# casper-hansen/AutoAWQ

Measured on NVIDIA H100. Metric: decode tok/s Llama-3-8B W4A16 (quantised linears, bs=1, seq=1), higher is better.
Workload: dtype f16

## Files before the change

### autoawq_b200/csrc/common.cuh

```cuda
#pragma once
#include <cuda_fp16.h>
#include <cuda_runtime.h>
#include <stdint.h>

namespace b200awq {

#ifndef B200AWQ_SM_COUNT_FALLBACK
#define B200AWQ_SM_COUNT_FALLBACK 132
#endif

__device__ __forceinline__ uint32_t smem_u32(const void* p) {
  return static_cast<uint32_t>(__cvta_generic_to_shared(p));
}
__device__ __forceinline__ uint32_t lane_id() { return threadIdx.x & 31; }

__device__ __forceinline__ bool elect_one() {
  uint32_t pred;
  asm volatile(
      "{\n\t.reg .pred p;\n\telect.sync _|p, 0xffffffff;\n\tselp.u32 %0, 1, 0, p;\n\t}\n"
      : "=r"(pred));
  return pred != 0;
}

__device__ __forceinline__ uint4 ldg_stream_u4(const void* p) {
// ... 154 lines not shown
  asm volatile("prefetch.tensormap [%0];" ::"l"(tmap) : "memory");
}
__device__ __forceinline__ void tma_load_2d(void* smem_dst, const void* tmap, uint64_t* bar, int c0, int c1) {
  asm volatile(
      "cp.async.bulk.tensor.2d.shared::cluster.global.mbarrier::complete_tx::bytes [%0], [%1, {%3, %4}], [%2];"
      ::"r"(smem_u32(smem_dst)), "l"(tmap), "r"(smem_u32(bar)), "r"(c0), "r"(c1)
      : "memory");
}
__device__ __forceinline__ void tma_prefetch_l2_2d(const void* tmap, int c0, int c1) {
  asm volatile("cp.async.bulk.prefetch.tensor.2d.L2.global [%0, {%1, %2}];" ::"l"(tmap), "r"(c0), "r"(c1) : "memory");
}
__device__ __forceinline__ void prefetch_l2_line(const void* gsrc) {
  asm volatile("prefetch.global.L2 [%0];" ::"l"(gsrc) : "memory");
}
__device__ __forceinline__ void bulk_prefetch_l2(const void* gsrc, uint32_t bytes) {
  asm volatile("cp.async.bulk.prefetch.L2.global [%0], %1;" ::"l"(gsrc), "r"(bytes) : "memory");
}
__device__ __forceinline__ void bulk_load_1d(void* smem_dst, const void* gsrc, uint32_t bytes, uint64_t* bar) {
  asm volatile(
      "cp.async.bulk.shared::cluster.global.mbarrier::complete_tx::bytes [%0], [%1], %2, [%3];"
      ::"r"(smem_u32(smem_dst)), "l"(gsrc), "r"(bytes), "r"(smem_u32(bar))
      : "memory");
}

__device__ __forceinline__ void wgmma_fence() { asm volatile("wgmma.fence.sync.aligned;" ::: "memory"); }
__device__ __forceinline__ void wgmma_commit() { asm volatile("wgmma.commit_group.sync.aligned;" ::: "memory"); }
template <int N>
__device__ __forceinline__ void wgmma_wait() { asm volatile("wgmma.wait_group.sync.aligned %0;" ::"n"(N) : "memory"); }

__device__ __forceinline__ uint64_t gmma_desc(uint32_t smem_addr, uint32_t lbo_bytes, uint32_t sbo_bytes) {
  uint64_t d = 0;
  d |= static_cast<uint64_t>((smem_addr & 0x3FFFFu) >> 4);
  d |= static_cast<uint64_t>((lbo_bytes >> 4) & 0x3FFFu) << 16;
  d |= static_cast<uint64_t>((sbo_bytes >> 4) & 0x3FFFu) << 32;
  d |= static_cast<uint64_t>(1) << 62;
  return d;
}

template <int TA>
__device__ __forceinline__ void wgmma_m64n16k16(float (&d)[8], uint64_t da, uint64_t db) {
  asm volatile(
      "wgmma.mma_async.sync.aligned.m64n16k16.f32.f16.f16 "
      "{%0, %1, %2, %3, %4, %5, %6, %7}, "
      "%8, %9, 1, 1, 1, %10, 0;"
      : "+f"(d[0]), "+f"(d[1]), "+f"(d[2]), "+f"(d[3]), "+f"(d[4]), "+f"(d[5]), "+f"(d[6]), "+f"(d[7])
      : "l"(da), "l"(db), "n"(TA)
// ... 44 lines not shown
```

### autoawq_b200/csrc/program.cu

```cuda
#include <algorithm>
#include <cstring>
#include <vector>

#include "../../include/b200awq.h"
#include "common.cuh"
#include "gemv_tile.cuh"
#include "kernels.h"
#include "rope.cuh"

namespace b200awq {

enum { kProCopy = 0, kProRmsnorm = 1, kProSilu = 2 };

struct ProgOp {
  const __half* scales;
  const int32_t* qzeros;
  const __half* bias;
  __half* y;
  const __half* src;
  const __half* norm_w;
  __half* xout;
  int src_off;
  int src_prev;
  int K, N, G;
// ... 68 lines not shown
  while (!mbar_try_wait(bar, parity))
    if (wd.tick(code, op)) return false;
  return true;
}

}
#include "program_stream.cuh"
#include "program_batch.cuh"
namespace b200awq {

struct Program {
  int n_ops = 0;
  int M = 0;
  size_t xs_bytes = 0;
  int device = 0;
  SpOp* d_sp_ops = nullptr;
  uint8_t* d_stream = nullptr;
  uint32_t* d_cta = nullptr;
  uint32_t* d_rows = nullptr;
  int* d_state = nullptr;
  int row_stride = 0;
  size_t stream_bytes = 0;
  int sb_spw = 0, sb_lmax = 0, sb_nu_max = 0;
  SpMoe* d_moe = nullptr;
  int n_moe = 0;
  SpRes* d_res = nullptr;
  SpRope* d_rope = nullptr;
};

struct ResFold {
  const void* raw_y = nullptr;
  const void* ext = nullptr;
  int op = -1;
};

struct MoeFold {
  int kind = 0;
  int mi = -1;
};

int moe_plan(int E, int topk, int H, int I, int G, int grid, int* out8) {
  if (E <= 0 || topk <= 0 || topk > E || H <= 0 || I <= 0 || G <= 0 || grid <= 0 || out8 == nullptr)
    return B200AWQ_EINVAL;
  if (E > kSpMoeEMax || topk > kSpMoeKMax) return B200AWQ_EUNSUPPORTED;
  if (!stream_format_supported(H, 2 * I, G, 1) || !stream_format_supported(I, H, G, 0)) return B200AWQ_EUNSUPPORTED;
  const int UK = G < 128 ? G : 128;
// ... 10 lines not shown
  out8[1] = sets_a;
  out8[2] = (2 * I / 16) * nu_a;
  out8[3] = lmax_a;
  out8[4] = topk * nu_b1;
  out8[5] = nu_b1;
  out8[6] = lmax_b;
  out8[7] = (int)smem;
  return B200AWQ_OK;
}

size_t stream_format_bytes(int K, int N, int G) {
  if (K <= 0 || N <= 0 || G <= 0) return 0;
  const int UK = G < 128 ? G : 128;
  return (size_t)(N / 16) * (K / UK) * ((size_t)(UK / 16) * 128 + kSpAux);
}
bool stream_format_supported(int K, int N, int G, int mode) {
  if (K <= 0 || N <= 0 || G <= 0 || (K % G) != 0 || (N % 16) != 0 || (K % 128) != 0) return false;
  if (!(G == 32 || G == 64 || (G % 128) == 0)) return false;
  if (mode == 1 && ((N / 2) % 8) != 0) return false;
  return mode == 0 || mode == 1;
}
static int prog_sm_count();

cudaError_t stream_pack_rotary(const int32_t* qweight, const void* scales, const int32_t* qzeros, void* out, int K, int N,
                               int G, int head_dim, cudaStream_t st) {
  if (!stream_format_supported(K, N, G, 0) || head_dim <= 0 || (head_dim % 16) != 0 || (N % head_dim) != 0)
    return cudaErrorNotSupported;
  const int UK = G < 128 ? G : 128;
  const int64_t total = (int64_t)(N / 16) * (K / UK) * ((UK / 16) * 32 + 12);
  const int cap = prog_sm_count() * 16;
  const int blocks = (int)((total + 255) / 256 < cap ? (total + 255) / 256 : cap);
  stream_pack_rotary_kernel<<<blocks, 256, 0, st>>>(qweight, static_cast<const __half*>(scales), qzeros,
                                                    static_cast<uint8_t*>(out), K, N, G, head_dim);
  return cudaGetLastError();
}

cudaError_t stream_pack(const int32_t* qweight, const void* scales, const int32_t* qzeros, void* out, int K, int N, int G,
                        int mode, cudaStream_t st) {
  if (!stream_format_supported(K, N, G, mode)) return cudaErrorNotSupported;
  const int UK = G < 128 ? G : 128;
  const int64_t total = (int64_t)(N / 16) * (K / UK) * ((UK / 16) * 32 + 12);
  const int cap = prog_sm_count() * 16;
  const int blocks = (int)((total + 255) / 256 < cap ? (total + 255) / 256 : cap);
  stream_pack_kernel<<<blocks, 256, 0, st>>>(qweight, static_cast<const __half*>(scales), qzeros,
                                             static_cast<uint8_t*>(out), K, N, G, mode);
  return cudaGetLastError();
// ... 47 lines not shown
      has_res = true;
    }
  size_t wbytes = 0, max_cols = 0;
  int max_K = 0, lmax = 0, nu_max = 0;
  std::vector<size_t> woff(n);
  for (int i = 0; i < n; ++i) {
    const ProgOp& p = table[i];
    if (moe_kind(i) != 0) {
      woff[i] = wbytes;
      wbytes += (size_t)moes[fold[i].mi].E * expert_bytes(i);
    } else {
      if (!stream_format_supported(p.K, p.N, p.G, mode[i] == 2 ? 0 : mode[i])) return false;
      const int UK = p.G < 128 ? p.G : 128;
      if (p.K / UK > kSpXsumMax) return false;
      if (M == 1 && (p.N / 16 + grid - 1) / grid > kSpLMax) return false;
      lmax = std::max(lmax, (p.N / 16 + grid - 1) / grid);
      nu_max = std::max(nu_max, p.K / UK);
      woff[i] = wbytes;
      wbytes += (stream_format_bytes(p.K, p.N, p.G) + 255) & ~(size_t)255;
    }
    max_cols = std::max(max_cols, (size_t)(mode[i] == 1 ? p.N / 2 : p.N));
    max_K = std::max(max_K, p.K);
  }
  if (M == 1 && (has_moe || has_res || has_rope)) {
    if (sp_fixed_smem(8, 4, true) + (size_t)max_K * 2 > (size_t)227 * 1024) return false;
  } else if (M == 1) {
    if (sp_fixed_smem(12, 3) + (size_t)max_K * 2 > (size_t)227 * 1024) return false;
  } else {
    int spw = kSbMaxStages;
    while (spw > 0 && sb_fixed_smem(spw, lmax, sb_mt(M), nu_max) + (size_t)max_K * sb_mt(M) * 2 > (size_t)227 * 1024) --spw;
    if (spw == 0) return false;
    pr->sb_spw = spw;
    pr->sb_lmax = lmax;
    pr->sb_nu_max = nu_max;
  }
  for (int i = 0; i < n; ++i) {
    const ProgOp& p = table[i];
    SpOp& o = ops[i];
    std::memset(&o, 0, sizeof(o));
    o.bias = p.bias;
    o.y = (!res.empty() && res[i].raw_y != nullptr) ? static_cast<__half*>(const_cast<void*>(res[i].raw_y)) : p.y;
    o.K = p.K;
    o.N = p.N;
    const int UK = p.G < 128 ? p.G : 128;
    o.uk_shift = UK == 32 ? 5 : (UK == 64 ? 6 : 7);
    o.F = UK / 16;
    o.NU = p.K / UK;
    o.unit_bytes = o.F * 128 + kSpAux;
    o.ups = kSpStageBytes / o.unit_bytes;
    o.mode = mode[i];
// ... 126 lines not shown
      e = cudaFuncSetAttribute(stream_batch_residual_kernel<2>, cudaFuncAttributeMaxDynamicSharedMemorySize, (int)(227 * 1024));
    if (e == cudaSuccess)
      e = cudaFuncSetAttribute(stream_batch_residual_kernel<4>, cudaFuncAttributeMaxDynamicSharedMemorySize, (int)(227 * 1024));
    if (e == cudaSuccess)
      e = cudaFuncSetAttribute(stream_batch_residual_kernel<8>, cudaFuncAttributeMaxDynamicSharedMemorySize, (int)(227 * 1024));
  }
  if (e == cudaSuccess && has_rope) {
    std::vector<SpRope> rp(n);
    for (int i = 0; i < n; ++i) rp[i].r = ropes[i];
    e = cudaMalloc(&pr->d_rope, (size_t)n * sizeof(SpRope));
    if (e == cudaSuccess) e = cudaMemcpy(pr->d_rope, rp.data(), (size_t)n * sizeof(SpRope), cudaMemcpyHostToDevice);
    if (e == cudaSuccess)
      e = cudaFuncSetAttribute(stream_rope_kernel, cudaFuncAttributeMaxDynamicSharedMemorySize, (int)(227 * 1024));
    if (e == cudaSuccess)
      e = cudaFuncSetAttribute(stream_batch_rope_kernel<2>, cudaFuncAttributeMaxDynamicSharedMemorySize, (int)(227 * 1024));
    if (e == cudaSuccess)
      e = cudaFuncSetAttribute(stream_batch_rope_kernel<4>, cudaFuncAttributeMaxDynamicSharedMemorySize, (int)(227 * 1024));
    if (e == cudaSuccess)
      e = cudaFuncSetAttribute(stream_batch_rope_kernel<8>, cudaFuncAttributeMaxDynamicSharedMemorySize, (int)(227 * 1024));
  }
  if (e == cudaSuccess) e = cudaMemcpy(pr->d_sp_ops, ops.data(), (size_t)n * sizeof(SpOp), cudaMemcpyHostToDevice);
  if (e == cudaSuccess) e = cudaMemcpy(pr->d_cta, cta.data(), cta.size() * sizeof(uint32_t), cudaMemcpyHostToDevice);
  if (e == cudaSuccess)
    e = cudaFuncSetAttribute(stream_program_kernel<8, 4, 4>, cudaFuncAttributeMaxDynamicSharedMemorySize, (int)(227 * 1024));
  if (e == cudaSuccess)
    e = cudaFuncSetAttribute(stream_program_kernel<12, 3, 2>, cudaFuncAttributeMaxDynamicSharedMemorySize, (int)(227 * 1024));
  if (e == cudaSuccess && M > 1) {
    e = cudaFuncSetAttribute(stream_batch_kernel<2>, cudaFuncAttributeMaxDynamicSharedMemorySize, (int)(227 * 1024));
    if (e == cudaSuccess)
      e = cudaFuncSetAttribute(stream_batch_kernel<4>, cudaFuncAttributeMaxDynamicSharedMemorySize, (int)(227 * 1024));
    if (e == cudaSuccess)
      e = cudaFuncSetAttribute(stream_batch_kernel<8>, cudaFuncAttributeMaxDynamicSharedMemorySize, (int)(227 * 1024));
  }
  if (e == cudaSuccess) e = cudaDeviceSynchronize();
  if (e != cudaSuccess) {
    cudaFree(pr->d_stream);
    cudaFree(pr->d_sp_ops);
    cudaFree(pr->d_cta);
    cudaFree(pr->d_rows);
    cudaFree(pr->d_state);
    cudaFree(pr->d_moe);
    cudaFree(pr->d_res);
    cudaFree(pr->d_rope);
    pr->d_res = nullptr;
    pr->d_rope = nullptr;
    pr->d_stream = nullptr;
    pr->d_sp_ops = nullptr;
    pr->d_cta = nullptr;
    pr->d_rows = nullptr;
// ... 390 lines not shown
    cfg.attrs = attr;
    cfg.numAttrs = 1;
    const SpOp* sops = p->d_sp_ops;
    const uint32_t* cta = p->d_cta;
    if (p->d_rope != nullptr) {
      auto qk = sb_mt(p->M) == 2 ? stream_batch_rope_kernel<2>
                                 : (sb_mt(p->M) == 4 ? stream_batch_rope_kernel<4> : stream_batch_rope_kernel<8>);
      const SpRes* rd = p->d_res;
      const SpRope* qd = p->d_rope;
      return cudaLaunchKernelEx(&cfg, qk, sops, cta, p->n_ops, p->d_rows, p->row_stride, p->d_state, p->M, p->sb_spw,
                                p->sb_lmax, p->sb_nu_max, knob(3), rd, qd);
    }
    if (p->d_res != nullptr) {
      auto rk = sb_mt(p->M) == 2 ? stream_batch_residual_kernel<2>
                                 : (sb_mt(p->M) == 4 ? stream_batch_residual_kernel<4> : stream_batch_residual_kernel<8>);
      const SpRes* rd = p->d_res;
      return cudaLaunchKernelEx(&cfg, rk, sops, cta, p->n_ops, p->d_rows, p->row_stride, p->d_state, p->M, p->sb_spw,
                                p->sb_lmax, p->sb_nu_max, knob(3), rd);
    }
    auto kern = sb_mt(p->M) == 2 ? stream_batch_kernel<2> : (sb_mt(p->M) == 4 ? stream_batch_kernel<4> : stream_batch_kernel<8>);
    return cudaLaunchKernelEx(&cfg, kern, sops, cta, p->n_ops, p->d_rows, p->row_stride, p->d_state, p->M, p->sb_spw,
                              p->sb_lmax, p->sb_nu_max, knob(3));
  }
  const int nw = knob(9) == 12 ? 12 : 8;
  const int spw = nw == 8 ? 4 : 3;
  cudaLaunchConfig_t cfg = {};
  cfg.gridDim = dim3(prog_sm_count());
  cfg.blockDim = dim3(32 + nw * 32);
  cfg.dynamicSmemBytes = sp_fixed_smem(nw, spw) + p->xs_bytes;
  cfg.stream = st;
  cudaLaunchAttribute attr[1];
  attr[0].id = cudaLaunchAttributeCooperative;
  attr[0].val.cooperative = 1;
  cfg.attrs = attr;
  cfg.numAttrs = 1;
  const SpOp* sops = p->d_sp_ops;
  const uint32_t* cta = p->d_cta;
  const int l2_ahead = knob(8) <= 0 ? 0 : knob(8) * 1024;
  const int gate_ahead = knob(10) <= 0 ? 1 << 20 : knob(10) - 1;
  const SpMoe* no_moe = nullptr;
  if (p->d_rope != nullptr) {
    cfg.blockDim = dim3(32 + 8 * 32);
    cfg.dynamicSmemBytes = sp_fixed_smem(8, 4, true) + p->xs_bytes;
    const SpMoe* md = p->d_moe;
    const SpRes* rd = p->d_res;
    const SpRope* qd = p->d_rope;
    return cudaLaunchKernelEx(&cfg, stream_rope_kernel, sops, cta, p->n_ops, p->d_rows, p->row_stride, p->d_state,
                              knob(3), l2_ahead, gate_ahead, md, rd, qd);
  }
  if (p->d_res != nullptr) {
    cfg.blockDim = dim3(32 + 8 * 32);
    cfg.dynamicSmemBytes = sp_fixed_smem(8, 4, true) + p->xs_bytes;
    const SpMoe* md = p->d_moe;
    const SpRes* rd = p->d_res;
    return cudaLaunchKernelEx(&cfg, stream_residual_kernel, sops, cta, p->n_ops, p->d_rows, p->row_stride, p->d_state,
                              knob(3), l2_ahead, gate_ahead, md, rd);
  }
  if (p->n_moe > 0) {
    cfg.blockDim = dim3(32 + 8 * 32);
    cfg.dynamicSmemBytes = sp_fixed_smem(8, 4, true) + p->xs_bytes;
    const SpMoe* md = p->d_moe;
    return cudaLaunchKernelEx(&cfg, stream_moe_kernel, sops, cta, p->n_ops, p->d_rows,
                              p->row_stride, p->d_state, knob(3), l2_ahead, gate_ahead, md);
  }
  if (nw == 8)
    return cudaLaunchKernelEx(&cfg, stream_program_kernel<8, 4, 4>, sops, cta, p->n_ops, p->d_rows, p->row_stride,
                              p->d_state, knob(3), l2_ahead, gate_ahead, no_moe);
  return cudaLaunchKernelEx(&cfg, stream_program_kernel<12, 3, 2>, sops, cta, p->n_ops, p->d_rows, p->row_stride,
                            p->d_state, knob(3), l2_ahead, gate_ahead, no_moe);
}

void program_destroy(Program* p) {
  if (p == nullptr) return;
  cudaFree(p->d_sp_ops);
  cudaFree(p->d_stream);
  cudaFree(p->d_cta);
  cudaFree(p->d_rows);
  cudaFree(p->d_state);
  cudaFree(p->d_moe);
  cudaFree(p->d_res);
  cudaFree(p->d_rope);
  delete p;
}

}
```

### autoawq_b200/csrc/program_stream.cuh

```cuda
#pragma once

namespace b200awq {

constexpr int kSpMaxWarps = 16;
constexpr int kSpStageWarps = 8;
constexpr int kSpStagePass = kSpStageWarps * 32 * 8;
constexpr int kSpStageBytes = 4288;
constexpr int kSpAux = 48;
constexpr int kSpLMax = 32;
constexpr int kSpRows = 4;
constexpr int kSpXsumMax = 1024;

struct __align__(128) SpOp {
  const uint8_t* wstream;
  const uint32_t* cta_begin;
  const __half* bias;
  __half* y;
  const __half* src;
  const __half* norm_w;
  __half* xout;
  __half* act_out;
  int K, N;
  int uk_shift, F, NU, unit_bytes, ups;
  int mode;
// ... 5 lines not shown
  int moe_i;
  int pad_[1];
};
static_assert(sizeof(SpOp) == 128, "SpOp layout");

constexpr int kSpMoeEMax = 64;
constexpr int kSpMoeKMax = 8;
constexpr int kSpMoeSmem = 512;
struct SpMoe {
  const __half* gate_w;
  __half* logits;
  float* topk_w;
  int* topk_ids;
  int* tok_idx;
  int* sorted_ids;
  int* expert_ids;
  int* npost;
  __half* down;
  long long eb_a, eb_b;
  int E, topk, renorm, block_size, sorted_len;
  int seg_a, seg_b, I;
};

__host__ __device__ constexpr size_t sp_fixed_smem(int nw, int spw, bool moe = false) {
  return (size_t)nw * spw * kSpStageBytes + (size_t)kSpLMax * nw * 16 * 4 + (size_t)kSpXsumMax * 4 +
         (size_t)2 * nw * spw * 8 + 2 * 128 + 256 + (moe ? kSpMoeSmem : 0);
}
static_assert(sp_fixed_smem(8, 4) % 16 == 0 && sp_fixed_smem(12, 3) % 16 == 0 && sp_fixed_smem(16, 2) % 16 == 0,
              "xs must stay 16-byte aligned");

__device__ __forceinline__ uint4 ld_relaxed_u4(const void* p) {
  uint4 r;
  asm volatile("ld.relaxed.gpu.global.v4.u32 {%0,%1,%2,%3}, [%4];" : "=r"(r.x), "=r"(r.y), "=r"(r.z), "=r"(r.w) : "l"(p) : "memory");
  return r;
}
__device__ __forceinline__ void st_relaxed_u32(void* p, uint32_t v) {
  asm volatile("st.relaxed.gpu.global.u32 [%0], %1;" ::"l"(p), "r"(v) : "memory");
}
__device__ __forceinline__ void st_release_cta_smem(int* p, int v) {
  asm volatile("st.release.cta.shared.s32 [%0], %1;" ::"r"(smem_u32(p)), "r"(v) : "memory");
}
__device__ __forceinline__ int ld_acquire_cta_smem(const int* p) {
  int v;
  asm volatile("ld.acquire.cta.shared.s32 %0, [%1];" : "=r"(v) : "r"(smem_u32(p)) : "memory");
  return v;
}
__device__ __forceinline__ uint32_t sp_tag(int base, int op) { return (uint32_t)((base + op) % 65535 + 1); }

constexpr int kSpResWindow = 4;
struct SpRes {
  const __half* ext;
// ... 223 lines not shown
__device__ __forceinline__ void cp_async_16(void* smem_dst, const void* gsrc) {
  asm volatile("cp.async.ca.shared.global [%0], [%1], 16;" ::"r"(smem_u32(smem_dst)), "l"(gsrc) : "memory");
}
__device__ __forceinline__ void cp_async_4(void* smem_dst, const void* gsrc) {
  asm volatile("cp.async.ca.shared.global [%0], [%1], 4;" ::"r"(smem_u32(smem_dst)), "l"(gsrc) : "memory");
}
__device__ __forceinline__ void cp_async_wait_all() { asm volatile("cp.async.wait_all;" ::: "memory"); }

struct SpMoeSmem {
  float* m_logit;
  float* m_w;
  int* m_ids;
  int* routed_op;
};
__device__ __forceinline__ SpMoeSmem sp_moe_smem(uint8_t* area) {
  SpMoeSmem s;
  s.m_logit = reinterpret_cast<float*>(area);
  s.m_w = s.m_logit + kSpMoeEMax;
  s.m_ids = reinterpret_cast<int*>(s.m_w + kSpMoeKMax);
  s.routed_op = s.m_ids + kSpMoeKMax;
  return s;
}

template <int NW, int SPW, int GR, bool MOE = false>
__global__ void __launch_bounds__(32 + NW * 32, 1)
    stream_program_kernel(const SpOp* __restrict__ ops, const uint32_t* __restrict__ cta_all, int n_ops,
                          uint32_t* __restrict__ rows, int row_stride, int* __restrict__ state, int dbg, int l2_ahead,
                          int gate_ahead, const SpMoe* __restrict__ moe) {
#include "program_stream_body.inc"
}

__global__ void __launch_bounds__(32 + 8 * 32, 1)
    stream_moe_kernel(const SpOp* __restrict__ ops, const uint32_t* __restrict__ cta_all, int n_ops,
                      uint32_t* __restrict__ rows, int row_stride, int* __restrict__ state, int dbg, int l2_ahead,
                      int gate_ahead, const SpMoe* __restrict__ moe) {
  constexpr int NW = 8, SPW = 4, GR = 4;
  constexpr bool MOE = true;
  pdl_wait();
#include "program_stream_body.inc"
}

__global__ void __launch_bounds__(32 + 8 * 32, 1)
    stream_residual_kernel(const SpOp* __restrict__ ops, const uint32_t* __restrict__ cta_all, int n_ops,
                           uint32_t* __restrict__ rows, int row_stride, int* __restrict__ state, int dbg, int l2_ahead,
                           int gate_ahead, const SpMoe* __restrict__ moe, const SpRes* __restrict__ res) {
  constexpr int NW = 8, SPW = 4, GR = 4;
  constexpr bool MOE = true;
  pdl_wait();
#define SP_RESIDUAL 1
#include "program_stream_body.inc"
#undef SP_RESIDUAL
}

__global__ void __launch_bounds__(32 + 8 * 32, 1)
    stream_rope_kernel(const SpOp* __restrict__ ops, const uint32_t* __restrict__ cta_all, int n_ops,
                       uint32_t* __restrict__ rows, int row_stride, int* __restrict__ state, int dbg, int l2_ahead,
                       int gate_ahead, const SpMoe* __restrict__ moe, const SpRes* __restrict__ res,
                       const SpRope* __restrict__ rope) {
  constexpr int NW = 8, SPW = 4, GR = 4;
  constexpr bool MOE = true;
  pdl_wait();
#define SP_RESIDUAL 1
#define SP_ROPE 1
#include "program_stream_body.inc"
#undef SP_ROPE
#undef SP_RESIDUAL
}

}
```

### autoawq_b200/csrc/program_stream_body.inc

```
  extern __shared__ __align__(1024) uint8_t sp_smem[];
  uint8_t* ring = sp_smem;
  float* part = reinterpret_cast<float*>(sp_smem + (size_t)(NW * SPW) * kSpStageBytes);
  float* xsum = part + kSpLMax * NW * 16;
  uint64_t* full = reinterpret_cast<uint64_t*>(xsum + kSpXsumMax);
  uint64_t* empty = full + (NW * SPW);
  SpOp* sdesc = reinterpret_cast<SpOp*>(empty + (NW * SPW));
  int* misc = reinterpret_cast<int*>(sdesc + 2);
  float* wsum = reinterpret_cast<float*>(misc);
  int* wfirst = misc + 8;
  int* wlast = misc + 8 + NW;
  uint32_t* scta = reinterpret_cast<uint32_t*>(misc + 8 + 2 * NW);
  int* staged_op = misc + 12 + 2 * NW;
  static_assert((13 + 2 * NW) * 4 <= 256, "misc area");
  uint32_t* xs = reinterpret_cast<uint32_t*>(sp_smem + sp_fixed_smem(NW, SPW, MOE));

  const int tid = threadIdx.x, warp = tid >> 5, lane = tid & 31;
  const int nblk = gridDim.x, bid = blockIdx.x;
  const int base = state[0];

  if (tid == 0) {
    for (int s = 0; s < (NW * SPW); ++s) {
      mbar_init(&full[s], 1);
      mbar_init(&empty[s], 1);
    }
    fence_mbar_init();
    *staged_op = -1;
    if constexpr (MOE) *sp_moe_smem(sp_smem + sp_fixed_smem(NW, SPW)).routed_op = -1;
  }
  if (warp == 1) {
    reinterpret_cast<uint32_t*>(sdesc)[lane] = reinterpret_cast<const uint32_t*>(ops)[lane];
    if (lane < 2) scta[lane] = cta_all[bid + lane];
  }
  __syncthreads();

  if (warp == 0) {
    if constexpr (MOE) {
      {
        const SpMoeSmem ms = sp_moe_smem(sp_smem + sp_fixed_smem(NW, SPW));
        const int* m_ids = ms.m_ids;
        const int* routed_op = ms.routed_op;
        const int w = lane < NW ? lane : 0;
        bool active = lane < NW;
        struct Run {
          uint32_t u, ub;
          int UB, ups;
          const uint8_t* src;
        };
        auto fetch = [&](int op, Run& r) {
          r.u = r.ub = 0;
          r.UB = r.ups = 1;
          r.src = nullptr;
          if (op < n_ops && lane < NW) {
            const uint32_t u0 = cta_all[(size_t)op * (nblk + 1) + bid], u1 = cta_all[(size_t)op * (nblk + 1) + bid + 1];
            const uint32_t nu = u1 - u0;
            r.u = u0 + (uint32_t)((uint64_t)nu * w / NW);
            r.ub = u0 + (uint32_t)((uint64_t)nu * (w + 1) / NW);
            r.UB = ops[op].unit_bytes;
            r.ups = ops[op].ups;
            r.src = ops[op].wstream;
          }
        };
// ... 50 lines not shown
        for (;;) {
          while (active && cur.u >= cur.ub) {
            if (++op >= n_ops) {
              active = false;
              break;
            }
            cur = nxt;
            fetch(op + 1, nxt);
            if constexpr (MOE) {
              mcur = mnxt;
              mfetch(op + 1, mnxt);
            }
          }
          if (!__any_sync(0xffffffffu, active)) break;
          bool issued = false;
          bool routed = true, route_wait = false;
          if constexpr (MOE) {
            if (active && mcur.kind != 0) {
              routed = ld_acquire_cta_smem(routed_op) >= mcur.need;
              route_wait = !routed;
            }
          }
          if (active && routed && (gate_ahead >= (1 << 20) || op <= ld_acquire_cta_smem(staged_op) + gate_ahead)) {
            const int stage = w * SPW + stage_i;
            if (mbar_test_wait(&empty[stage], ph ^ 1)) {
              if constexpr (MOE) {
                int n = (int)(cur.ub - cur.u) < cur.ups ? (int)(cur.ub - cur.u) : cur.ups;
                const uint8_t* src = cur.src + (size_t)cur.u * cur.UB;
                if (mcur.kind != 0) src = mchunk(cur, mcur, n);
                mbar_arrive_expect_tx(&full[stage], (uint32_t)(n * cur.UB));
                bulk_load_1d(ring + (size_t)stage * kSpStageBytes, src, (uint32_t)(n * cur.UB), &full[stage]);
                cur.u += (uint32_t)n;
                ahead -= n * cur.UB;
              } else {
                const int n = (int)(cur.ub - cur.u) < cur.ups ? (int)(cur.ub - cur.u) : cur.ups;
                mbar_arrive_expect_tx(&full[stage], (uint32_t)(n * cur.UB));
                bulk_load_1d(ring + (size_t)stage * kSpStageBytes, cur.src + (size_t)cur.u * cur.UB, (uint32_t)(n * cur.UB),
                             &full[stage]);
                cur.u += (uint32_t)cur.ups;
                ahead -= n * cur.UB;
              }
              if (++stage_i == SPW) { stage_i = 0; ph ^= 1; }
              issued = true;
            }
          }
          if (!__any_sync(0xffffffffu, issued)) {
            bool pf = false;
            if (pactive) {
              if (ahead < 0) {
                pop = op;
                pcur = cur;
                pnxt = nxt;
                if constexpr (MOE) {
                  mpcur = mcur;
                  mpnxt = mnxt;
                }
                ahead = 0;
              }
              while (pactive && pcur.u >= pcur.ub) {
                if (++pop >= n_ops) {
                  pactive = false;
                  break;
                }
                pcur = pnxt;
                fetch(pop + 1, pnxt);
                if constexpr (MOE) {
                  mpcur = mpnxt;
                  mfetch(pop + 1, mpnxt);
                }
              }
              if constexpr (MOE) {
                if (pactive && ahead < l2_ahead && (mpcur.kind == 0 || ld_acquire_cta_smem(routed_op) == mpcur.need)) {
                  int n = (int)(pcur.ub - pcur.u) < pcur.ups ? (int)(pcur.ub - pcur.u) : pcur.ups;
                  const uint8_t* src = pcur.src + (size_t)pcur.u * pcur.UB;
                  if (mpcur.kind != 0) src = mchunk(pcur, mpcur, n);
                  bulk_prefetch_l2(src, (uint32_t)(n * pcur.UB));
                  pcur.u += (uint32_t)n;
                  ahead += n * pcur.UB;
                  pf = true;
                }
              } else {
                if (pactive && ahead < l2_ahead) {
                  const int n = (int)(pcur.ub - pcur.u) < pcur.ups ? (int)(pcur.ub - pcur.u) : pcur.ups;
                  bulk_prefetch_l2(pcur.src + (size_t)pcur.u * pcur.UB, (uint32_t)(n * pcur.UB));
                  pcur.u += (uint32_t)pcur.ups;
                  ahead += n * pcur.UB;
                  pf = true;
                }
              }
            }
            if (!__any_sync(0xffffffffu, pf)) {
              int code = kWEmpty;
              if constexpr (MOE) code = __any_sync(0xffffffffu, route_wait) ? kWRoute : kWEmpty;
              if (__any_sync(0xffffffffu, wd.tick(code, op))) break;
              __nanosleep(32);
            }
          }
        }
      }
    } else {
      {
        const int w = lane < NW ? lane : 0;
        bool active = lane < NW;
        struct Run {
          uint32_t u, ub;
          int UB, ups;
          const uint8_t* src;
// ... 17 lines not shown
        fetch(0, cur);
        fetch(1, nxt);
        Run pcur, pnxt;
        int pop = 0;
        fetch(0, pcur);
        fetch(1, pnxt);
        bool pactive = lane < NW && l2_ahead > 0;
        int ahead = 0;
        int stage_i = 0;
        uint32_t ph = 0;
        ProgWatch wd;
        for (;;) {
          while (active && cur.u >= cur.ub) {
            if (++op >= n_ops) {
              active = false;
              break;
            }
            cur = nxt;
            fetch(op + 1, nxt);
          }
          if (!__any_sync(0xffffffffu, active)) break;
          bool issued = false;
          if (active && (gate_ahead >= (1 << 20) || op <= ld_acquire_cta_smem(staged_op) + gate_ahead)) {
            const int stage = w * SPW + stage_i;
            if (mbar_test_wait(&empty[stage], ph ^ 1)) {
              const int n = (int)(cur.ub - cur.u) < cur.ups ? (int)(cur.ub - cur.u) : cur.ups;
              mbar_arrive_expect_tx(&full[stage], (uint32_t)(n * cur.UB));
              bulk_load_1d(ring + (size_t)stage * kSpStageBytes, cur.src + (size_t)cur.u * cur.UB, (uint32_t)(n * cur.UB),
                           &full[stage]);
              cur.u += (uint32_t)cur.ups;
              ahead -= n * cur.UB;
              if (++stage_i == SPW) { stage_i = 0; ph ^= 1; }
              issued = true;
            }
          }
          if (!__any_sync(0xffffffffu, issued)) {
            bool pf = false;
            if (pactive) {
              if (ahead < 0) {
                pop = op;
                pcur = cur;
                pnxt = nxt;
                ahead = 0;
              }
              while (pactive && pcur.u >= pcur.ub) {
                if (++pop >= n_ops) {
                  pactive = false;
                  break;
                }
                pcur = pnxt;
                fetch(pop + 1, pnxt);
              }
              if (pactive && ahead < l2_ahead) {
                const int n = (int)(pcur.ub - pcur.u) < pcur.ups ? (int)(pcur.ub - pcur.u) : pcur.ups;
                bulk_prefetch_l2(pcur.src + (size_t)pcur.u * pcur.UB, (uint32_t)(n * pcur.UB));
                pcur.u += (uint32_t)pcur.ups;
                ahead += n * pcur.UB;
                pf = true;
              }
            }
            if (!__any_sync(0xffffffffu, pf)) {
              if (__any_sync(0xffffffffu, wd.tick(kWEmpty, op))) break;
              __nanosleep(32);
            }
          }
        }
      }
    }
  } else {
    const int cw = warp - 1;
    const int ct = tid - 32;
    const int g = lane >> 2, tig = lane & 3;
    const bool xl = g == 0;
    int stage_i = 0;
    uint32_t ph = 0;

    for (int op = 0; op < n_ops; ++op) {
      const SpOp* o = sdesc + (op & 1);
// ... 121 lines not shown
                const uint4 wv = cb0 == cb_first ? nwv[b] : __ldg(reinterpret_cast<const uint4*>(nw + c));
#pragma unroll
                for (int q = 0; q < 4; ++q) {
                  const float2 a = __half22float2(u32_as_h2(dst[2 * q]));
                  const float2 wq = __half22float2(u32_as_h2((&wv.x)[q]));
                  h[q] = h2_as_u32(__halves2half2(__float2half_rn(a.x * rs * wq.x), __float2half_rn(a.y * rs * wq.y)));
                  dst[2 * q] = h[q];
                }
                if (c >= xlo && c < xhi) *reinterpret_cast<uint4*>(xout + c) = make_uint4(h[0], h[1], h[2], h[3]);
              }
              unit_sums(c, ok, h);
            }
          }
        }
        named_bar_sync_gv(1, (NW * 32));
      }
      if (ct == 0) st_release_cta_smem(staged_op, op);
      SP_STAMP(2);
      SP_TOUCH_SMEM();
      SP_WSTAMP(2);
      if constexpr (MOE) {
        if (o->moe == 1) {
          const SpMoe* md = moe + o->moe_i;
          const SpMoeSmem ms = sp_moe_smem(sp_smem + sp_fixed_smem(NW, SPW));
          float* m_logit = ms.m_logit;
          float* m_w = ms.m_w;
          int* m_ids = ms.m_ids;
          const int E = md->E, topk = md->topk;
          for (int e = cw; e < E; e += NW) {
            const __half* wr = md->gate_w + (size_t)e * K;
            float d = 0.f;
#pragma unroll 4
            for (int c = lane * 8; c < K; c += 256) {
              const uint4 wv = __ldg(reinterpret_cast<const uint4*>(wr + c));
              const uint32_t* xp = xs + (c >> 4) * 8 + ((c >> 3) & 1);
#pragma unroll
              for (int q = 0; q < 4; ++q) {
                const float2 a = __half22float2(u32_as_h2(xp[2 * q]));
                const float2 b = __half22float2(u32_as_h2((&wv.x)[q]));
                d = fmaf(a.x, b.x, d);
                d = fmaf(a.y, b.y, d);
              }
            }
            d = prog_warp_sum(d);
            if (lane == 0) m_logit[e] = __half2float(__float2half_rn(d));
          }
          named_bar_sync_gv(1, (NW * 32));
// ... 109 lines not shown
          float ylo = 0.f, yhi = 0.f;
          int first_ls = -1, last_ls = -1;
          auto flush = [&]() {
            const int ls = s_cur - set0c;
            if (tig == 0) {
              float* p = part + ((size_t)ls * NW + cw) * 16;
              p[g] = ylo;
              p[g + 8] = yhi;
            }
            if (first_ls < 0) first_ls = ls;
            last_ls = ls;
            ylo = yhi = 0.f;
          };
          int n_adv = ups;
          for (uint32_t u = ua; u < ub; u += (uint32_t)n_adv) {
            int n = (int)(ub - u) < ups ? (int)(ub - u) : ups;
            if constexpr (MOE) {
              if (mseg != 0) {
                const int rr = (int)(u % (uint32_t)mseg);
                if (mseg - rr < n) n = mseg - rr;
                n_adv = n;
              }
            }
            const int stage = cw * SPW + stage_i;
            prog_mbar_wait(&full[stage], ph, kWFull, op);
            if (u == ua) {
              SP_STAMP(3);
              SP_WSTAMP(3);
            }
            const uint8_t* st = ring + (size_t)stage * kSpStageBytes;
            if (dbg != 5 && dbg != 7) {
              auto apply = [&](float t_lo, float t_hi) {
                ylo += t_lo;
                yhi += t_hi;
                if (++j == NUc) {
                  flush();
                  j = 0;
                  ++s_cur;
                }
              };
              int j0 = j;
              if constexpr (MOE) {
                if (o->moe == 2) j0 = (s_cur % mtopk) * NUc + j;
              }
              if (F == 8) sp_chunk<8, GR>(st, UB, n, xs, xsum, j0, NU, lane, xl, apply);
              else if (F == 4) sp_chunk<4, GR>(st, UB, n, xs, xsum, j0, NU, lane, xl, apply);
              else sp_chunk<2, GR>(st, UB, n, xs, xsum, j0, NU, lane, xl, apply);
            }
            __syncwarp();
            if (lane == 0) mbar_arrive(&empty[stage]);
            if (++stage_i == SPW) { stage_i = 0; ph ^= 1; }
          }
          if (j != 0 && ua < ub) flush();
          if (lane == 0) {
            wfirst[cw] = first_ls;
            wlast[cw] = last_ls;
          }
        }
      } else {
        {
          int s_cur = (int)(ua / NU), j = (int)(ua - (uint32_t)s_cur * NU);
          float ylo = 0.f, yhi = 0.f;
          int first_ls = -1, last_ls = -1;
          auto flush = [&]() {
            const int ls = s_cur - set0;
            if (tig == 0) {
              float* p = part + ((size_t)ls * NW + cw) * 16;
              p[g] = ylo;
              p[g + 8] = yhi;
            }
            if (first_ls < 0) first_ls = ls;
            last_ls = ls;
            ylo = yhi = 0.f;
          };
          for (uint32_t u = ua; u < ub; u += ups) {
            const int n = (int)(ub - u) < ups ? (int)(ub - u) : ups;
            const int stage = cw * SPW + stage_i;
            prog_mbar_wait(&full[stage], ph, kWFull, op);
            if (u == ua) {
              SP_STAMP(3);
              SP_WSTAMP(3);
            }
            const uint8_t* st = ring + (size_t)stage * kSpStageBytes;
            if (dbg != 5 && dbg != 7) {
              auto apply = [&](float t_lo, float t_hi) {
                ylo += t_lo;
                yhi += t_hi;
                if (++j == NU) {
                  flush();
                  j = 0;
                  ++s_cur;
                }
              };
              const int j0 = j;
              if (F == 8) sp_chunk<8, GR>(st, UB, n, xs, xsum, j0, NU, lane, xl, apply);
              else if (F == 4) sp_chunk<4, GR>(st, UB, n, xs, xsum, j0, NU, lane, xl, apply);
              else sp_chunk<2, GR>(st, UB, n, xs, xsum, j0, NU, lane, xl, apply);
            }
            __syncwarp();
            if (lane == 0) mbar_arrive(&empty[stage]);
            if (++stage_i == SPW) { stage_i = 0; ph ^= 1; }
          }
          if (j != 0 && ua < ub) flush();
          if (lane == 0) {
            wfirst[cw] = first_ls;
            wlast[cw] = last_ls;
          }
        }
      }
      SP_STAMP(4);
      SP_WSTAMP(4);
      if (cw == 0) cp_async_wait_all();
      named_bar_sync_gv(1, (NW * 32));
      SP_STAMP(5);
      SP_TOUCH_SMEM();
      SP_WSTAMP(5);

      if constexpr (MOE) {
#if SP_RESIDUAL
        const SpRes rs = res[op];
#endif
        bool moe_done = false;
        {
          if (o->moe != 0) {
            const SpMoe* md = moe + o->moe_i;
            const float* m_w = sp_moe_smem(sp_smem + sp_fixed_smem(NW, SPW)).m_w;
            const int topk = md->topk, I = md->I;
            const int nsets = nu == 0 ? 0 : (int)((u1 - 1) / NU) - set0 + 1;
            const uint32_t tagw = sp_tag(base, op) << 16;
            uint32_t* out_row = rows + (size_t)(op % kSpRows) * row_stride;
            for (int t = ct; t < nsets * 8; t += (NW * 32)) {
              const int ls = t >> 3, gg = t & 7;
              int clo, chi;
              sp_cols(mode, N, set0 + ls, gg, clo, chi);
              if (o->moe == 1) {
                float lo = 0.f, hi = 0.f;
  #pragma unroll
                for (int w = 0; w < NW; ++w) {
                  if (wfirst[w] >= 0 && wfirst[w] <= ls && ls <= wlast[w]) {
                    const float* p = part + ((size_t)ls * NW + w) * 16;
                    lo += p[gg];
                    hi += p[gg + 8];
                  }
                }
                const __half hlo = __float2half_rn(lo), hhi = __float2half_rn(hi);
                const float gf = __half2float(hlo), uf = __half2float(hhi);
                const __half a = __float2half_rn(gf / (1.f + __expf(-gf)) * uf);
                st_relaxed_u32(out_row + clo, tagw | __half_as_ushort(a));
                if (act_out != nullptr) act_out[clo] = a;
// ... 156 lines not shown
```

Baseline: 550.9.

## Size stream ring depth at runtime, add L2 cache hints, rescale prefetch window

```diff
diff --git a/autoawq_b200/csrc/common.cuh b/autoawq_b200/csrc/common.cuh
--- a/autoawq_b200/csrc/common.cuh
+++ b/autoawq_b200/csrc/common.cuh
@@ -200,6 +200,27 @@
       ::"r"(smem_u32(smem_dst)), "l"(gsrc), "r"(bytes), "r"(smem_u32(bar))
       : "memory");
 }
+__device__ __forceinline__ uint64_t l2_policy_evict_first() {
+  uint64_t p;
+  asm volatile("createpolicy.fractional.L2::evict_first.b64 %0, 1.0;" : "=l"(p));
+  return p;
+}
+__device__ __forceinline__ uint64_t l2_policy_evict_last() {
+  uint64_t p;
+  asm volatile("createpolicy.fractional.L2::evict_last.b64 %0, 1.0;" : "=l"(p));
+  return p;
+}
+__device__ __forceinline__ void bulk_prefetch_l2_hint(const void* gsrc, uint32_t bytes, uint64_t policy) {
+  asm volatile("cp.async.bulk.prefetch.L2.global.L2::cache_hint [%0], %1, %2;" ::"l"(gsrc), "r"(bytes), "l"(policy)
+               : "memory");
+}
+__device__ __forceinline__ void bulk_load_1d_hint(void* smem_dst, const void* gsrc, uint32_t bytes, uint64_t* bar,
+                                                  uint64_t policy) {
+  asm volatile(
+      "cp.async.bulk.shared::cluster.global.mbarrier::complete_tx::bytes.L2::cache_hint [%0], [%1], %2, [%3], %4;"
+      ::"r"(smem_u32(smem_dst)), "l"(gsrc), "r"(bytes), "r"(smem_u32(bar)), "l"(policy)
+      : "memory");
+}
 
 __device__ __forceinline__ void wgmma_fence() { asm volatile("wgmma.fence.sync.aligned;" ::: "memory"); }
 __device__ __forceinline__ void wgmma_commit() { asm volatile("wgmma.commit_group.sync.aligned;" ::: "memory"); }
diff --git a/autoawq_b200/csrc/program.cu b/autoawq_b200/csrc/program.cu
--- a/autoawq_b200/csrc/program.cu
+++ b/autoawq_b200/csrc/program.cu
@@ -114,6 +114,8 @@
   int row_stride = 0;
   size_t stream_bytes = 0;
   int sb_spw = 0, sb_lmax = 0, sb_nu_max = 0;
+  int sp_spw8 = 0, sp_spw12 = 0;
+  int l2_bytes = 0;
   SpMoe* d_moe = nullptr;
   int n_moe = 0;
   SpRes* d_res = nullptr;
@@ -170,6 +172,12 @@
 }
 static int prog_sm_count();
 
+static int sp_pick_spw(int nw, bool moe, size_t xs_bytes) {
+  int spw = kSpMaxStages;
+  while (spw > 1 && sp_fixed_smem(nw, spw, moe) + xs_bytes > (size_t)227 * 1024) --spw;
+  return spw;
+}
+
 cudaError_t stream_pack_rotary(const int32_t* qweight, const void* scales, const int32_t* qzeros, void* out, int K, int N,
                                int G, int head_dim, cudaStream_t st) {
   if (!stream_format_supported(K, N, G, 0) || head_dim <= 0 || (head_dim % 16) != 0 || (N % head_dim) != 0)
@@ -263,10 +271,12 @@
     max_cols = std::max(max_cols, (size_t)(mode[i] == 1 ? p.N / 2 : p.N));
     max_K = std::max(max_K, p.K);
   }
-  if (M == 1 && (has_moe || has_res || has_rope)) {
-    if (sp_fixed_smem(8, 4, true) + (size_t)max_K * 2 > (size_t)227 * 1024) return false;
-  } else if (M == 1) {
-    if (sp_fixed_smem(12, 3) + (size_t)max_K * 2 > (size_t)227 * 1024) return false;
+  if (M == 1) {
+    const bool moe_k = has_moe || has_res || has_rope;
+    if (moe_k && sp_fixed_smem(8, 4, true) + (size_t)max_K * 2 > (size_t)227 * 1024) return false;
+    if (!moe_k && sp_fixed_smem(12, 3, false) + (size_t)max_K * 2 > (size_t)227 * 1024) return false;
+    pr->sp_spw8 = sp_pick_spw(8, moe_k, (size_t)max_K * 2);
+    pr->sp_spw12 = moe_k ? 0 : sp_pick_spw(12, false, (size_t)max_K * 2);
   } else {
     int spw = kSbMaxStages;
     while (spw > 0 && sb_fixed_smem(spw, lmax, sb_mt(M), nu_max) + (size_t)max_K * sb_mt(M) * 2 > (size_t)227 * 1024) --spw;
@@ -439,9 +449,10 @@
   if (e == cudaSuccess) e = cudaMemcpy(pr->d_sp_ops, ops.data(), (size_t)n * sizeof(SpOp), cudaMemcpyHostToDevice);
   if (e == cudaSuccess) e = cudaMemcpy(pr->d_cta, cta.data(), cta.size() * sizeof(uint32_t), cudaMemcpyHostToDevice);
   if (e == cudaSuccess)
-    e = cudaFuncSetAttribute(stream_program_kernel<8, 4, 4>, cudaFuncAttributeMaxDynamicSharedMemorySize, (int)(227 * 1024));
+    e = cudaFuncSetAttribute(stream_program_kernel<8, 4>, cudaFuncAttributeMaxDynamicSharedMemorySize, (int)(227 * 1024));
   if (e == cudaSuccess)
-    e = cudaFuncSetAttribute(stream_program_kernel<12, 3, 2>, cudaFuncAttributeMaxDynamicSharedMemorySize, (int)(227 * 1024));
+    e = cudaFuncSetAttribute(stream_program_kernel<12, 2>, cudaFuncAttributeMaxDynamicSharedMemorySize, (int)(227 * 1024));
+  if (e == cudaSuccess) e = cudaDeviceGetAttribute(&pr->l2_bytes, cudaDevAttrL2CacheSize, pr->device);
   if (e == cudaSuccess && M > 1) {
     e = cudaFuncSetAttribute(stream_batch_kernel<2>, cudaFuncAttributeMaxDynamicSharedMemorySize, (int)(227 * 1024));
     if (e == cudaSuccess)
@@ -878,12 +889,14 @@
     return cudaLaunchKernelEx(&cfg, kern, sops, cta, p->n_ops, p->d_rows, p->row_stride, p->d_state, p->M, p->sb_spw,
                               p->sb_lmax, p->sb_nu_max, knob(3));
   }
-  const int nw = knob(9) == 12 ? 12 : 8;
-  const int spw = nw == 8 ? 4 : 3;
+  const bool moe_k = p->d_rope != nullptr || p->d_res != nullptr || p->n_moe > 0;
+  const int nw = knob(9) == 12 && !moe_k ? 12 : 8;
+  const int spw = nw == 8 ? p->sp_spw8 : p->sp_spw12;
+  const int grid = prog_sm_count();
   cudaLaunchConfig_t cfg = {};
-  cfg.gridDim = dim3(prog_sm_count());
+  cfg.gridDim = dim3(grid);
   cfg.blockDim = dim3(32 + nw * 32);
-  cfg.dynamicSmemBytes = sp_fixed_smem(nw, spw) + p->xs_bytes;
+  cfg.dynamicSmemBytes = sp_fixed_smem(nw, spw, moe_k) + p->xs_bytes;
   cfg.stream = st;
   cudaLaunchAttribute attr[1];
   attr[0].id = cudaLaunchAttributeCooperative;
@@ -892,38 +905,33 @@
   cfg.numAttrs = 1;
   const SpOp* sops = p->d_sp_ops;
   const uint32_t* cta = p->d_cta;
-  const int l2_ahead = knob(8) <= 0 ? 0 : knob(8) * 1024;
+  const size_t window = knob(8) <= 0 ? 0 : std::min((size_t)knob(8) << 20, (size_t)p->l2_bytes);
+  const int l2_ahead = (int)(window / ((size_t)grid * nw));
   const int gate_ahead = knob(10) <= 0 ? 1 << 20 : knob(10) - 1;
   const SpMoe* no_moe = nullptr;
   if (p->d_rope != nullptr) {
-    cfg.blockDim = dim3(32 + 8 * 32);
-    cfg.dynamicSmemBytes = sp_fixed_smem(8, 4, true) + p->xs_bytes;
     const SpMoe* md = p->d_moe;
     const SpRes* rd = p->d_res;
     const SpRope* qd = p->d_rope;
-    return cudaLaunchKernelEx(&cfg, stream_rope_kernel, sops, cta, p->n_ops, p->d_rows, p->row_stride, p->d_state,
+    return cudaLaunchKernelEx(&cfg, stream_rope_kernel, sops, cta, p->n_ops, p->d_rows, p->row_stride, p->d_state, spw,
                               knob(3), l2_ahead, gate_ahead, md, rd, qd);
   }
   if (p->d_res != nullptr) {
-    cfg.blockDim = dim3(32 + 8 * 32);
-    cfg.dynamicSmemBytes = sp_fixed_smem(8, 4, true) + p->xs_bytes;
     const SpMoe* md = p->d_moe;
     const SpRes* rd = p->d_res;
     return cudaLaunchKernelEx(&cfg, stream_residual_kernel, sops, cta, p->n_ops, p->d_rows, p->row_stride, p->d_state,
-                              knob(3), l2_ahead, gate_ahead, md, rd);
+                              spw, knob(3), l2_ahead, gate_ahead, md, rd);
   }
   if (p->n_moe > 0) {
-    cfg.blockDim = dim3(32 + 8 * 32);
-    cfg.dynamicSmemBytes = sp_fixed_smem(8, 4, true) + p->xs_bytes;
     const SpMoe* md = p->d_moe;
-    return cudaLaunchKernelEx(&cfg, stream_moe_kernel, sops, cta, p->n_ops, p->d_rows,
-                              p->row_stride, p->d_state, knob(3), l2_ahead, gate_ahead, md);
+    return cudaLaunchKernelEx(&cfg, stream_moe_kernel, sops, cta, p->n_ops, p->d_rows, p->row_stride, p->d_state, spw,
+                              knob(3), l2_ahead, gate_ahead, md);
   }
   if (nw == 8)
-    return cudaLaunchKernelEx(&cfg, stream_program_kernel<8, 4, 4>, sops, cta, p->n_ops, p->d_rows, p->row_stride,
-                              p->d_state, knob(3), l2_ahead, gate_ahead, no_moe);
-  return cudaLaunchKernelEx(&cfg, stream_program_kernel<12, 3, 2>, sops, cta, p->n_ops, p->d_rows, p->row_stride,
-                            p->d_state, knob(3), l2_ahead, gate_ahead, no_moe);
+    return cudaLaunchKernelEx(&cfg, stream_program_kernel<8, 4>, sops, cta, p->n_ops, p->d_rows, p->row_stride,
+                              p->d_state, spw, knob(3), l2_ahead, gate_ahead, no_moe);
+  return cudaLaunchKernelEx(&cfg, stream_program_kernel<12, 2>, sops, cta, p->n_ops, p->d_rows, p->row_stride,
+                            p->d_state, spw, knob(3), l2_ahead, gate_ahead, no_moe);
 }
 
 void program_destroy(Program* p) {
diff --git a/autoawq_b200/csrc/program_stream.cuh b/autoawq_b200/csrc/program_stream.cuh
--- a/autoawq_b200/csrc/program_stream.cuh
+++ b/autoawq_b200/csrc/program_stream.cuh
@@ -51,11 +51,15 @@
   int seg_a, seg_b, I;
 };
 
-__host__ __device__ constexpr size_t sp_fixed_smem(int nw, int spw, bool moe = false) {
-  return (size_t)nw * spw * kSpStageBytes + (size_t)kSpLMax * nw * 16 * 4 + (size_t)kSpXsumMax * 4 +
-         (size_t)2 * nw * spw * 8 + 2 * 128 + 256 + (moe ? kSpMoeSmem : 0);
-}
-static_assert(sp_fixed_smem(8, 4) % 16 == 0 && sp_fixed_smem(12, 3) % 16 == 0 && sp_fixed_smem(16, 2) % 16 == 0,
+constexpr int kSpMaxStages = 8;
+constexpr int kSpMoeOff = 512;
+__host__ __device__ constexpr size_t sp_ring_off(int nw, bool moe) {
+  return kSpMoeOff + (moe ? kSpMoeSmem : 0) + (size_t)kSpLMax * nw * 16 * 4 + (size_t)kSpXsumMax * 4;
+}
+__host__ __device__ constexpr size_t sp_fixed_smem(int nw, int spw, bool moe) {
+  return sp_ring_off(nw, moe) + (size_t)nw * spw * (kSpStageBytes + 2 * 8);
+}
+static_assert(sp_fixed_smem(8, 4, false) % 16 == 0 && sp_fixed_smem(12, 3, true) % 16 == 0,
               "xs must stay 16-byte aligned");
 
 __device__ __forceinline__ uint4 ld_relaxed_u4(const void* p) {
@@ -325,19 +329,19 @@
   return s;
 }
 
-template <int NW, int SPW, int GR, bool MOE = false>
+template <int NW, int GR, bool MOE = false>
 __global__ void __launch_bounds__(32 + NW * 32, 1)
     stream_program_kernel(const SpOp* __restrict__ ops, const uint32_t* __restrict__ cta_all, int n_ops,
-                          uint32_t* __restrict__ rows, int row_stride, int* __restrict__ state, int dbg, int l2_ahead,
-                          int gate_ahead, const SpMoe* __restrict__ moe) {
+                          uint32_t* __restrict__ rows, int row_stride, int* __restrict__ state, int spw, int dbg,
+                          int l2_ahead, int gate_ahead, const SpMoe* __restrict__ moe) {
 #include "program_stream_body.inc"
 }
 
 __global__ void __launch_bounds__(32 + 8 * 32, 1)
     stream_moe_kernel(const SpOp* __restrict__ ops, const uint32_t* __restrict__ cta_all, int n_ops,
-                      uint32_t* __restrict__ rows, int row_stride, int* __restrict__ state, int dbg, int l2_ahead,
-                      int gate_ahead, const SpMoe* __restrict__ moe) {
-  constexpr int NW = 8, SPW = 4, GR = 4;
+                      uint32_t* __restrict__ rows, int row_stride, int* __restrict__ state, int spw, int dbg,
+                      int l2_ahead, int gate_ahead, const SpMoe* __restrict__ moe) {
+  constexpr int NW = 8, GR = 4;
   constexpr bool MOE = true;
   pdl_wait();
 #include "program_stream_body.inc"
@@ -345,9 +349,9 @@
 
 __global__ void __launch_bounds__(32 + 8 * 32, 1)
     stream_residual_kernel(const SpOp* __restrict__ ops, const uint32_t* __restrict__ cta_all, int n_ops,
-                           uint32_t* __restrict__ rows, int row_stride, int* __restrict__ state, int dbg, int l2_ahead,
-                           int gate_ahead, const SpMoe* __restrict__ moe, const SpRes* __restrict__ res) {
-  constexpr int NW = 8, SPW = 4, GR = 4;
+                           uint32_t* __restrict__ rows, int row_stride, int* __restrict__ state, int spw, int dbg,
+                           int l2_ahead, int gate_ahead, const SpMoe* __restrict__ moe, const SpRes* __restrict__ res) {
+  constexpr int NW = 8, GR = 4;
   constexpr bool MOE = true;
   pdl_wait();
 #define SP_RESIDUAL 1
@@ -357,10 +361,10 @@
 
 __global__ void __launch_bounds__(32 + 8 * 32, 1)
     stream_rope_kernel(const SpOp* __restrict__ ops, const uint32_t* __restrict__ cta_all, int n_ops,
-                       uint32_t* __restrict__ rows, int row_stride, int* __restrict__ state, int dbg, int l2_ahead,
-                       int gate_ahead, const SpMoe* __restrict__ moe, const SpRes* __restrict__ res,
+                       uint32_t* __restrict__ rows, int row_stride, int* __restrict__ state, int spw, int dbg,
+                       int l2_ahead, int gate_ahead, const SpMoe* __restrict__ moe, const SpRes* __restrict__ res,
                        const SpRope* __restrict__ rope) {
-  constexpr int NW = 8, SPW = 4, GR = 4;
+  constexpr int NW = 8, GR = 4;
   constexpr bool MOE = true;
   pdl_wait();
 #define SP_RESIDUAL 1
diff --git a/autoawq_b200/csrc/program_stream_body.inc b/autoawq_b200/csrc/program_stream_body.inc
--- a/autoawq_b200/csrc/program_stream_body.inc
+++ b/autoawq_b200/csrc/program_stream_body.inc
@@ -1,31 +1,31 @@
   extern __shared__ __align__(1024) uint8_t sp_smem[];
-  uint8_t* ring = sp_smem;
-  float* part = reinterpret_cast<float*>(sp_smem + (size_t)(NW * SPW) * kSpStageBytes);
+  SpOp* sdesc = reinterpret_cast<SpOp*>(sp_smem);
+  int* misc = reinterpret_cast<int*>(sdesc + 2);
+  float* part = reinterpret_cast<float*>(sp_smem + kSpMoeOff + (MOE ? kSpMoeSmem : 0));
   float* xsum = part + kSpLMax * NW * 16;
-  uint64_t* full = reinterpret_cast<uint64_t*>(xsum + kSpXsumMax);
-  uint64_t* empty = full + (NW * SPW);
-  SpOp* sdesc = reinterpret_cast<SpOp*>(empty + (NW * SPW));
-  int* misc = reinterpret_cast<int*>(sdesc + 2);
+  uint8_t* ring = sp_smem + sp_ring_off(NW, MOE);
+  uint64_t* full = reinterpret_cast<uint64_t*>(ring + (size_t)NW * spw * kSpStageBytes);
+  uint64_t* empty = full + NW * spw;
   float* wsum = reinterpret_cast<float*>(misc);
   int* wfirst = misc + 8;
   int* wlast = misc + 8 + NW;
   uint32_t* scta = reinterpret_cast<uint32_t*>(misc + 8 + 2 * NW);
   int* staged_op = misc + 12 + 2 * NW;
   static_assert((13 + 2 * NW) * 4 <= 256, "misc area");
-  uint32_t* xs = reinterpret_cast<uint32_t*>(sp_smem + sp_fixed_smem(NW, SPW, MOE));
+  uint32_t* xs = reinterpret_cast<uint32_t*>(sp_smem + sp_fixed_smem(NW, spw, MOE));
 
   const int tid = threadIdx.x, warp = tid >> 5, lane = tid & 31;
   const int nblk = gridDim.x, bid = blockIdx.x;
   const int base = state[0];
 
   if (tid == 0) {
-    for (int s = 0; s < (NW * SPW); ++s) {
+    for (int s = 0; s < NW * spw; ++s) {
       mbar_init(&full[s], 1);
       mbar_init(&empty[s], 1);
     }
     fence_mbar_init();
     *staged_op = -1;
-    if constexpr (MOE) *sp_moe_smem(sp_smem + sp_fixed_smem(NW, SPW)).routed_op = -1;
+    if constexpr (MOE) *sp_moe_smem(sp_smem + kSpMoeOff).routed_op = -1;
   }
   if (warp == 1) {
     reinterpret_cast<uint32_t*>(sdesc)[lane] = reinterpret_cast<const uint32_t*>(ops)[lane];
@@ -36,7 +36,7 @@
   if (warp == 0) {
     if constexpr (MOE) {
       {
-        const SpMoeSmem ms = sp_moe_smem(sp_smem + sp_fixed_smem(NW, SPW));
+        const SpMoeSmem ms = sp_moe_smem(sp_smem + kSpMoeOff);
         const int* m_ids = ms.m_ids;
         const int* routed_op = ms.routed_op;
         const int w = lane < NW ? lane : 0;
@@ -133,25 +133,26 @@
             }
           }
           if (active && routed && (gate_ahead >= (1 << 20) || op <= ld_acquire_cta_smem(staged_op) + gate_ahead)) {
-            const int stage = w * SPW + stage_i;
+            const int stage = stage_i * NW + w;
             if (mbar_test_wait(&empty[stage], ph ^ 1)) {
               if constexpr (MOE) {
                 int n = (int)(cur.ub - cur.u) < cur.ups ? (int)(cur.ub - cur.u) : cur.ups;
                 const uint8_t* src = cur.src + (size_t)cur.u * cur.UB;
                 if (mcur.kind != 0) src = mchunk(cur, mcur, n);
                 mbar_arrive_expect_tx(&full[stage], (uint32_t)(n * cur.UB));
-                bulk_load_1d(ring + (size_t)stage * kSpStageBytes, src, (uint32_t)(n * cur.UB), &full[stage]);
+                bulk_load_1d_hint(ring + (size_t)stage * kSpStageBytes, src, (uint32_t)(n * cur.UB), &full[stage],
+                                  l2_policy_evict_first());
                 cur.u += (uint32_t)n;
                 ahead -= n * cur.UB;
               } else {
                 const int n = (int)(cur.ub - cur.u) < cur.ups ? (int)(cur.ub - cur.u) : cur.ups;
                 mbar_arrive_expect_tx(&full[stage], (uint32_t)(n * cur.UB));
-                bulk_load_1d(ring + (size_t)stage * kSpStageBytes, cur.src + (size_t)cur.u * cur.UB, (uint32_t)(n * cur.UB),
-                             &full[stage]);
+                bulk_load_1d_hint(ring + (size_t)stage * kSpStageBytes, cur.src + (size_t)cur.u * cur.UB,
+                                  (uint32_t)(n * cur.UB), &full[stage], l2_policy_evict_first());
                 cur.u += (uint32_t)cur.ups;
                 ahead -= n * cur.UB;
               }
-              if (++stage_i == SPW) { stage_i = 0; ph ^= 1; }
+              if (++stage_i == spw) { stage_i = 0; ph ^= 1; }
               issued = true;
             }
           }
@@ -185,7 +186,7 @@
                   int n = (int)(pcur.ub - pcur.u) < pcur.ups ? (int)(pcur.ub - pcur.u) : pcur.ups;
                   const uint8_t* src = pcur.src + (size_t)pcur.u * pcur.UB;
                   if (mpcur.kind != 0) src = mchunk(pcur, mpcur, n);
-                  bulk_prefetch_l2(src, (uint32_t)(n * pcur.UB));
+                  bulk_prefetch_l2_hint(src, (uint32_t)(n * pcur.UB), l2_policy_evict_last());
                   pcur.u += (uint32_t)n;
                   ahead += n * pcur.UB;
                   pf = true;
@@ -193,7 +194,8 @@
               } else {
                 if (pactive && ahead < l2_ahead) {
                   const int n = (int)(pcur.ub - pcur.u) < pcur.ups ? (int)(pcur.ub - pcur.u) : pcur.ups;
-                  bulk_prefetch_l2(pcur.src + (size_t)pcur.u * pcur.UB, (uint32_t)(n * pcur.UB));
+                  bulk_prefetch_l2_hint(pcur.src + (size_t)pcur.u * pcur.UB, (uint32_t)(n * pcur.UB),
+                                        l2_policy_evict_last());
                   pcur.u += (uint32_t)pcur.ups;
                   ahead += n * pcur.UB;
                   pf = true;
@@ -257,15 +259,15 @@
           if (!__any_sync(0xffffffffu, active)) break;
           bool issued = false;
           if (active && (gate_ahead >= (1 << 20) || op <= ld_acquire_cta_smem(staged_op) + gate_ahead)) {
-            const int stage = w * SPW + stage_i;
+            const int stage = stage_i * NW + w;
             if (mbar_test_wait(&empty[stage], ph ^ 1)) {
               const int n = (int)(cur.ub - cur.u) < cur.ups ? (int)(cur.ub - cur.u) : cur.ups;
               mbar_arrive_expect_tx(&full[stage], (uint32_t)(n * cur.UB));
-              bulk_load_1d(ring + (size_t)stage * kSpStageBytes, cur.src + (size_t)cur.u * cur.UB, (uint32_t)(n * cur.UB),
-                           &full[stage]);
+              bulk_load_1d_hint(ring + (size_t)stage * kSpStageBytes, cur.src + (size_t)cur.u * cur.UB,
+                                (uint32_t)(n * cur.UB), &full[stage], l2_policy_evict_first());
               cur.u += (uint32_t)cur.ups;
               ahead -= n * cur.UB;
-              if (++stage_i == SPW) { stage_i = 0; ph ^= 1; }
+              if (++stage_i == spw) { stage_i = 0; ph ^= 1; }
               issued = true;
             }
           }
@@ -288,7 +290,8 @@
               }
               if (pactive && ahead < l2_ahead) {
                 const int n = (int)(pcur.ub - pcur.u) < pcur.ups ? (int)(pcur.ub - pcur.u) : pcur.ups;
-                bulk_prefetch_l2(pcur.src + (size_t)pcur.u * pcur.UB, (uint32_t)(n * pcur.UB));
+                bulk_prefetch_l2_hint(pcur.src + (size_t)pcur.u * pcur.UB, (uint32_t)(n * pcur.UB),
+                                      l2_policy_evict_last());
                 pcur.u += (uint32_t)pcur.ups;
                 ahead += n * pcur.UB;
                 pf = true;
@@ -456,7 +459,7 @@
       if constexpr (MOE) {
         if (o->moe == 1) {
           const SpMoe* md = moe + o->moe_i;
-          const SpMoeSmem ms = sp_moe_smem(sp_smem + sp_fixed_smem(NW, SPW));
+          const SpMoeSmem ms = sp_moe_smem(sp_smem + kSpMoeOff);
           float* m_logit = ms.m_logit;
           float* m_w = ms.m_w;
           int* m_ids = ms.m_ids;
@@ -612,7 +615,7 @@
                 n_adv = n;
               }
             }
-            const int stage = cw * SPW + stage_i;
+            const int stage = stage_i * NW + cw;
             prog_mbar_wait(&full[stage], ph, kWFull, op);
             if (u == ua) {
               SP_STAMP(3);
@@ -639,7 +642,7 @@
             }
             __syncwarp();
             if (lane == 0) mbar_arrive(&empty[stage]);
-            if (++stage_i == SPW) { stage_i = 0; ph ^= 1; }
+            if (++stage_i == spw) { stage_i = 0; ph ^= 1; }
           }
           if (j != 0 && ua < ub) flush();
           if (lane == 0) {
@@ -665,7 +668,7 @@
           };
           for (uint32_t u = ua; u < ub; u += ups) {
             const int n = (int)(ub - u) < ups ? (int)(ub - u) : ups;
-            const int stage = cw * SPW + stage_i;
+            const int stage = stage_i * NW + cw;
             prog_mbar_wait(&full[stage], ph, kWFull, op);
             if (u == ua) {
               SP_STAMP(3);
@@ -689,7 +692,7 @@
             }
             __syncwarp();
             if (lane == 0) mbar_arrive(&empty[stage]);
-            if (++stage_i == SPW) { stage_i = 0; ph ^= 1; }
+            if (++stage_i == spw) { stage_i = 0; ph ^= 1; }
           }
           if (j != 0 && ua < ub) flush();
           if (lane == 0) {
@@ -714,7 +717,7 @@
         {
           if (o->moe != 0) {
             const SpMoe* md = moe + o->moe_i;
-            const float* m_w = sp_moe_smem(sp_smem + sp_fixed_smem(NW, SPW)).m_w;
+            const float* m_w = sp_moe_smem(sp_smem + kSpMoeOff).m_w;
             const int topk = md->topk, I = md->I;
             const int nsets = nu == 0 ? 0 : (int)((u1 - 1) / NU) - set0 + 1;
             const uint32_t tagw = sp_tag(base, op) << 16;
```

Result: faster. 572.9, median of 6 (+4.0%).
